# ioloizou/g1_locomotion

Hardware: AMD Instinct MI355X
Metric: QP solves/sec, SRBD N=10 12-state/12-input (higher is better)
Workload: dtype f64; 1 GPU; configs[1]: batch=4096/GPU random SRBD states, N=10, 2-contact alternating single support friction cone, fp64; tails deferred (SRBDQP_FLAG_DEFER_TAIL: the ~4 % of a batch that reach a rho-restart mark finish in the next launch on their stream; srbdqp_flush inside the timed region, every batch complete when the clock stops); steps rotate over 4 distinct device batches; horizon=10, batch_per_gpu=4096, kernel=wave_defer_f64_n10_s2, streams=2, longest_first_hint=False, deferred_tails=True, world_size=1, distinct_batches=4, max_iter=250, rho_restart_iter=0, rho_restart_count=0, set_up_dtype=f64

## Files before the change

g1_locomotion_amd/csrc/srbdqp_mfma.hpp:

```cpp
#pragma once
#include "srbdqp_common.hpp"
#include "srbdqp_admm.hpp"

namespace srbdqp {

constexpr bool kMfmaReady = true;

#ifdef SRBDQP_PROFILE_F
#define F_T(var) do { unsigned long long t_; asm volatile("s_memtime %0\n\ts_waitcnt lgkmcnt(0)" : "=s"(t_) :: "memory"); var = (long long)t_; } while (0)
#else
#define F_T(var) do { } while (0)
#endif

typedef double v4d __attribute__((ext_vector_type(4)));

__device__ __forceinline__ v4d mfma_f64(double a, double b, v4d c) {
    return __builtin_amdgcn_mfma_f64_16x16x4f64(a, b, c, 0, 0, 0);
}

__device__ __forceinline__ double readlane_f64(double v, int lane) {
    const int lo = __builtin_amdgcn_readlane(__double2loint(v), lane);
    const int hi = __builtin_amdgcn_readlane(__double2hiint(v), lane);
    return __hiloint2double(hi, lo);
}

__device__ __forceinline__ int tile_id(int a, int b) { return (b * (b + 1)) / 2 + a; }

template <bool SWZ>
__device__ __forceinline__ void store_tile(double* tile, const v4d& v, int lane) {
    const int col = lane & 15, g = lane >> 4;
#pragma unroll
    for (int r = 0; r < 4; ++r) {
        const int row = g + 4 * r;
        tile[row * 16 + (SWZ ? (col ^ row) : col)] = v[r];
    }
}

typedef float v4f __attribute__((ext_vector_type(4)));
__device__ __forceinline__ v4d mma16(double a, double b, v4d c) { return __builtin_amdgcn_mfma_f64_16x16x4f64(a, b, c, 0, 0, 0); }
__device__ __forceinline__ v4f mma16(float a, float b, v4f c) { return __builtin_amdgcn_mfma_f32_16x16x4f32(a, b, c, 0, 0, 0); }
template <typename TT> __device__ __forceinline__ int crow(int kq, int q) { return (sizeof(TT) == 8) ? kq + 4 * q : 4 * kq + q; }
template <typename TT, bool SWZ, typename V4>
__device__ __forceinline__ void store_tile_t(TT* tile, const V4& v, int lane) {
    const int col = lane & 15, g = lane >> 4;
#pragma unroll
    for (int q = 0; q < 4; ++q) {
        const int row = crow<TT>(g, q);
        tile[row * 16 + (SWZ ? (col ^ row) : col)] = v[q];
    }
}

__device__ __forceinline__ double fast_rsqrt(double d) {
    const double r = __builtin_amdgcn_rsq(d);
    const double h = 0.5 * d * r;
    return fma(r, fma(-h, r, 0.5), r);
}

__device__ __forceinline__ double fast_rsqrt2(double d) {
    double r = __builtin_amdgcn_rsq(d);
    double h = 0.5 * d * r;
    r = fma(r, fma(-h, r, 0.5), r);
    h = 0.5 * d * r;
    return fma(r, fma(-h, r, 0.5), r);
}

template <int KB>
__device__ __forceinline__ void diag16_block(v4d& s, v4d& rr, v4d& w, double& pmin, int lane) {
    const int col = lane & 15, k = lane >> 4, li = col & 3;
    const double sk = s[KB];
    const double d00 = readlane_f64(sk, 4 * KB), d01 = readlane_f64(sk, 4 * KB + 1), d02 = readlane_f64(sk, 4 * KB + 2), d03 = readlane_f64(sk, 4 * KB + 3);
    const double d11 = readlane_f64(sk, 16 + 4 * KB + 1), d12 = readlane_f64(sk, 16 + 4 * KB + 2), d13 = readlane_f64(sk, 16 + 4 * KB + 3);
    const double d22 = readlane_f64(sk, 32 + 4 * KB + 2), d23 = readlane_f64(sk, 32 + 4 * KB + 3);
    const double d33 = readlane_f64(sk, 48 + 4 * KB + 3);
    const double x00 = fast_rsqrt(d00);
    const double r01 = d01 * x00, r02 = d02 * x00, r03 = d03 * x00;
    const double p1 = fma(-r01, r01, d11);
    const double x11 = fast_rsqrt(p1);
    const double r12 = fma(-r01, r02, d12) * x11, r13 = fma(-r01, r03, d13) * x11;
    const double p2 = fma(-r12, r12, fma(-r02, r02, d22));
    const double x22 = fast_rsqrt(p2);
    const double r23 = fma(-r12, r13, fma(-r02, r03, d23)) * x22;
    const double p3 = fma(-r23, r23, fma(-r13, r13, fma(-r03, r03, d33)));
    const double x33 = fast_rsqrt(p3);
    pmin = (d00 > 0.0 && p1 > 0.0 && p2 > 0.0 && p3 > 0.0) ? pmin : -1.0;
    const double x01 = -x00 * r01 * x11;
    const double x12 = -x11 * r12 * x22;
    const double x23 = -x22 * r23 * x33;
    const double x02 = -fma(x00, r02, x01 * r12) * x22;
    const double x13 = -fma(x11, r13, x12 * r23) * x33;
    const double x03 = -fma(x00, r03, fma(x01, r13, x02 * r23)) * x33;
    const double c0 = x00;
    const double c1 = (k == 0) ? x01 : x11;
    const double c2 = (k == 0) ? x02 : (k == 1) ? x12 : x22;
    const double c3 = (k == 0) ? x03 : (k == 1) ? x13 : (k == 2) ? x23 : x33;
    double a = (li == 0) ? c0 : (li == 1) ? c1 : (li == 2) ? c2 : c3;
    a = (k <= li) ? a : 0.0;
    const v4d zero = (v4d){0.0, 0.0, 0.0, 0.0};
    double u = mfma_f64(a, sk, zero)[KB];
    u = (col >= 4 * KB) ? u : 0.0;
    const double wk = mfma_f64(a, rr[KB], zero)[KB];
    w[KB] = wk;
    if constexpr (KB < 3) {
        s = mfma_f64(-u, u, s);
        const double am = (col >= 4 * (KB + 1)) ? u : 0.0;
        rr = mfma_f64(-am, wk, rr);
        diag16_block<KB + 1>(s, rr, w, pmin, lane);
    }
}

__device__ __forceinline__ v4d diag16_invert_mfma(v4d s, int lane, bool& ok) {
    const int col = lane & 15, g = lane >> 4;
    v4d rr, w;
#pragma unroll
    for (int r = 0; r < 4; ++r) { rr[r] = (g + 4 * r == col) ? 1.0 : 0.0; w[r] = 0.0; }
    double pmin = 1.0e300;
    diag16_block<0>(s, rr, w, pmin, lane);
    ok = pmin > 0.0;
    return w;
}


template <int I>
__device__ __forceinline__ void fmac_newbcast(double& acc, double nu, double m) {
    asm("v_fmac_f64_dpp %0, %1, %2 row_newbcast:%3 row_mask:0xf bank_mask:0xf" : "+v"(acc) : "v"(nu), "v"(m), "n"(I));
}
template <int K>
__device__ __forceinline__ double mov_newbcast(double v) {
    double d;
    asm("s_nop 1\n\tv_mov_b64_dpp %0, %1 row_newbcast:%2 row_mask:0xf bank_mask:0xf" : "=v"(d) : "v"(v), "n"(K));
    return d;
}
template <int K, int I>
struct Diag16Rows {
    static __device__ __forceinline__ void run(double (&S)[16], double (&R)[16], double nu, double u, double wk) {
        if constexpr (I < 16) {
            fmac_newbcast<I>(S[I], nu, u);
            fmac_newbcast<I>(R[I], nu, wk);
            Diag16Rows<K, I + 1>::run(S, R, nu, u, wk);
        }
    }
};
template <int K, int KEND = 16>
__device__ __forceinline__ void diag16_pivot(double (&S)[16], double (&R)[16], bool& ok) {
    const double d = mov_newbcast<K>(S[K]);
    ok = ok && (d > 0.0);
    const double r = fast_rsqrt(d);
    const double u = S[K] * r;
    const double wk = R[K] * r;
    R[K] = wk;
    if constexpr (K < 15) {
        double nu;
        asm("v_mul_f64 %0, %1, %2\n\ts_nop 1" : "=v"(nu) : "v"(S[K]), "v"(-r));
        Diag16Rows<K, K + 1>::run(S, R, nu, u, wk);
    }
    if constexpr (K + 1 < KEND) diag16_pivot<K + 1, KEND>(S, R, ok);
}
__device__ __forceinline__ v4d diag16_invert_dpp(v4d s, int lane, bool& ok, double* tile) {
    const int col = lane & 15, g = lane >> 4;
    asm volatile("" ::: "memory");
#pragma unroll
    for (int r = 0; r < 4; ++r) tile[(g + 4 * r) * 16 + col] = s[r];
    asm volatile("" ::: "memory");
    double S[16], R[16];
#pragma unroll
    for (int i = 0; i < 16; ++i) { S[i] = tile[i * 16 + col]; R[i] = (i == col) ? 1.0 : 0.0; }
    asm volatile("" ::: "memory");
    ok = true;
    diag16_pivot<0>(S, R, ok);
    if (g == 0) {
#pragma unroll
        for (int i = 0; i < 16; ++i) tile[i * 16 + (col ^ i)] = R[i];
    }
    asm volatile("" ::: "memory");
    v4d w;
#pragma unroll
    for (int q = 0; q < 4; ++q) { const int row = g + 4 * q; w[q] = tile[row * 16 + (col ^ row)]; }
    asm volatile("" ::: "memory");
    return w;
}
template <typename TI, typename TO>
__device__ __forceinline__ void diag16_invert_dpp_tiles(const TI* in, TO* out, int lane, bool& ok) {
    const int col = lane & 15, g = lane >> 4;
    double S[16], R[16];
#pragma unroll
    for (int i = 0; i < 16; ++i) { S[i] = (double)in[i * 16 + col]; R[i] = (i == col) ? 1.0 : 0.0; }
    asm volatile("s_waitcnt lgkmcnt(0)" ::: "memory");
    ok = true;
    diag16_pivot<0>(S, R, ok);
    if (g == 0) {
#pragma unroll
        for (int i = 0; i < 16; ++i) out[i * 16 + (col ^ i)] = (TO)R[i];
    }
    asm volatile("" ::: "memory");
}

}
```

g1_locomotion_amd/csrc/srbdqp_setup1.hpp:

```cpp
#pragma once
#include "srbdqp_split.hpp"

namespace srbdqp {

#ifdef SRBDQP_WAVE_STAMPS
#define WSTAMP(a, b, idx) SRBDQP_STAMP(a, b, idx)
#define WSTAMP_RT(a, b, idx) do { if ((a).stamps && threadIdx.x == 0) (a).stamps[(size_t)(b) * 16 + (idx)] = (long long)__builtin_amdgcn_s_memrealtime(); } while (0)
#else
#define WSTAMP(a, b, idx) do { } while (0)
#define WSTAMP_RT(a, b, idx) do { } while (0)
#endif

template <int N, int MAXS>
struct Setup1Smem {
    using S = CompactSmem<N, MAXS>;
    static constexpr int n = Dims<N>::n;
    static constexpr int up2(int v) { return (v + 1) & ~1; }
    static constexpr int o_x0 = S::o_x0, o_tm = S::o_tm, o_J = S::o_J;
    static constexpr int o_cp = S::o_R;
    static constexpr int o_mt = o_cp + up2(9 * N);
    static constexpr int o_ab = o_mt + 18 * N;
    static constexpr int o_gv = o_mt + up2(9 * S::NPAIR);
    static constexpr int o_t1 = o_gv + up2(9 * N);
    static constexpr int o_t2 = o_t1 + up2(9 * N);
    static constexpr int o_x0c = o_t1;
    static constexpr int o_tf = o_x0c + up2(S::nmax) + 16;
    static constexpr int endT = (o_t2 + up2(9 * N) > o_tf + 6 * N) ? o_t2 + up2(9 * N) : o_tf + 6 * N;
    static constexpr int o_xref = up2(endT);
    static constexpr int o_foot = o_xref + up2(N * 13);
    static constexpr int o_pcom = o_foot + N * 12;
    static constexpr int o_eh = o_foot;
    static constexpr int o_gx = o_foot;
    static constexpr int o_scr = o_xref;
    static constexpr int endIn = o_pcom + up2(N * 3);
    static constexpr int endIn2 = (endIn > o_scr + 258) ? endIn : o_scr + 258;
    static constexpr int kStgRow = 18;
    static constexpr int kStgTile = 16 * kStgRow;
    static constexpr int endStg = (endIn2 > o_cp + S::NT * kStgTile) ? endIn2 : o_cp + S::NT * kStgTile;
    static constexpr int endAb = o_ab + 16 * S::NT * kAbStride;
    static constexpr int o_end = endStg > endAb ? endStg : endAb;
    static constexpr size_t bytes = (size_t)o_end * sizeof(double);
    static constexpr bool supported = SplitWs<N, MAXS>::supported && S::NT <= 4;
    static_assert(n + 6 * N <= o_end - o_eh || true, "");
};

template <int N, int MAXS, bool FUSED, bool DUMP, bool PHI, int RP>
__device__ __forceinline__ bool setup1_pass(const KArgs& a, const QpIo& io, const int b, double* sm, double& rho_b, int& rs_pass, int& rs_done) {
    using S = CompactSmem<N, MAXS>;
    using W = SplitWs<N, MAXS>;
    using L1 = Setup1Smem<N, MAXS>;
    constexpr int n = Dims<N>::n, m = Dims<N>::m, NT = S::NT;
    int lane = threadIdx.x;
    if constexpr (RP == 2) asm volatile("" : "+v"(lane));
    [[maybe_unused]] double* const park = sm + L1::o_end;
    int mcol = lane & 15, kq = lane >> 4;
    double* ws = FUSED ? nullptr : a.ws + (size_t)b * W::doubles;
    int* icnt = reinterpret_cast<int*>(sm + S::o_int);
    int* imisc = icnt + 2 * N;
    uint8_t* act = reinterpret_cast<uint8_t*>(imisc + 8);
    uint8_t* sct = reinterpret_cast<uint8_t*>(sm + S::o_ct);
    const double* SQ = sm + S::o_sq;
    const double* CP = sm + L1::o_cp;

    WSTAMP(a, b, 0);
    WSTAMP_RT(a, b, 12);
    constexpr int JT = (12 * N + 63) / 64;
    double yc, ys;
    [[maybe_unused]] double v_xr[JT];
    if constexpr (RP == 2) {
        const int k = lane < N ? lane : 0;
        yc = sm[S::o_tm + k * 9 + 0];
        ys = sm[S::o_tm + k * 9 + 1];
    } else {
        const double* gx0 = io.x0 + (size_t)b * 13;
        const double* gxr = io.xref + (size_t)b * N * 13;
        const double* gft = io.foot + (size_t)b * N * 12;
        const uint8_t* gct = io.contact + (size_t)b * N * 4;
        const double* gpc = io.pcom ? io.pcom + (size_t)b * N * 3 : nullptr;
        const double v_x0 = gx0[lane < 13 ? lane : 0];
        const uint8_t v_ct = gct[lane < 4 * N ? lane : 0];
        const double v_yaw = gxr[(lane < N ? lane : 0) * 13 + 2];
        double v_f[JT][3], v_p[JT][3];
#pragma unroll
        for (int t = 0; t < JT; ++t) {
            const int tt = (lane + 64 * t < 12 * N) ? lane + 64 * t : 0;
            const int k = tt / 12, ci = (tt % 12) / 3;
            const double* pc = gpc ? gpc + k * 3 : gxr + k * 13 + 3;
#pragma unroll
            for (int c = 0; c < 3; ++c) { v_f[t][c] = gft[k * 12 + 3 * ci + c]; v_p[t][c] = pc[c]; }
            v_xr[t] = gxr[k * 13 + (tt - 12 * k)];
        }
        sincos(v_yaw, &ys, &yc);
        if (lane < 13) sm[S::o_x0 + lane] = v_x0;
        if (lane >= 32 && lane < 44) sm[S::o_sq + lane - 32] = a.sqrtq[lane - 32];
        if (lane < N * 4) sct[lane] = v_ct ? 1 : 0;
        if (lane < N) {
            double* T = sm + S::o_tm + lane * 9;
            T[0] = yc;  T[1] = ys;  T[2] = 0.0;
            T[3] = -ys; T[4] = yc;  T[5] = 0.0;
            T[6] = 0.0; T[7] = 0.0; T[8] = 1.0;
        }
        {
            const bool flag = (lane < 4 * N) && v_ct != 0;
            const unsigned long long bal = __ballot(flag);
            if (flag) act[__popcll(bal & ((1ull << lane) - 1ull))] = (uint8_t)lane;
            if (lane < N) icnt[lane] = __popcll(bal & ((4 * (lane + 1) >= 64) ? ~0ull : ((1ull << (4 * (lane + 1))) - 1ull)));
            const bool over = lane < N && __popcll((bal >> (4 * (lane < N ? lane : 0))) & 0xFull) > MAXS;
            const unsigned long long viol = __ballot(over);
            if (lane == 0) {
                imisc[0] = __popcll(bal);
                imisc[1] = viol != 0ull;
                sm[S::o_misc] = 0.0;
                sm[S::o_misc + 1] = 0.0;
            }
        }
#pragma unroll
        for (int t = 0; t < JT; ++t) {
            const int tt = lane + 64 * t;
            const int k = (tt < 12 * N ? tt : 0) / 12, cc = tt - 12 * k, ax = cc % 3;
            const double cs = __shfl(yc, k), sn = __shfl(ys, k);
            const double i0 = a.iinv[0], i1 = a.iinv[1], i2 = a.iinv[2];
            const double w00 = cs * cs * i0 + sn * sn * i1, w01 = cs * sn * (i0 - i1), w11 = sn * sn * i0 + cs * cs * i1;
            const double rx = v_f[t][0] - v_p[t][0];
            const double ry = v_f[t][1] - v_p[t][1];
            const double rz = v_f[t][2] - v_p[t][2];
            const double s0 = (ax == 0) ? 0.0 : ((ax == 1) ? -rz : ry);
            const double s1 = (ax == 0) ? rz : ((ax == 1) ? 0.0 : -rx);
            const double s2 = (ax == 0) ? -ry : ((ax == 1) ? rx : 0.0);
            if (tt < 12 * N) {
                double* J = sm + S::o_J + k * 36;
                J[0 * 12 + cc] = w00 * s0 + w01 * s1;
                J[1 * 12 + cc] = w01 * s0 + w11 * s1;
                J[2 * 12 + cc] = i2 * s2;
            }
        }
    }
    double ccu[N], csu[N], ccm = 0.0, csm = 0.0;
    {
        double ac = 0.0, as = 0.0;
#pragma unroll
        for (int k = 0; k < N; ++k) {
            const double c = lane_bcast(yc, k), s = lane_bcast(ys, k);
            ac += c;
            as += s;
            ccu[k] = ac;
            csu[k] = as;
            ccm += (k <= lane) ? c : 0.0;
            csm += (k <= lane) ? s : 0.0;
        }
    }
    if (lane < N) {
        double* C = sm + L1::o_cp + lane * 9;
        C[0] = ccm;  C[1] = csm; C[2] = 0.0;
        C[3] = -csm; C[4] = ccm; C[5] = 0.0;
        C[6] = 0.0;  C[7] = 0.0; C[8] = (double)(lane + 1);
    }
    __syncthreads();
    const int na = imisc[0];
    const int n_eff = 3 * na;
    double* xs0 = sm + L1::o_mt;
    static_assert(L1::o_end - L1::o_mt >= n + 12 * N, "early-exit scratch");
    if (RP != 2 && (imisc[1] != 0 || na == 0)) {
        if constexpr (DUMP) { if (lane == 0) a.ub_out[(size_t)b * m] = (imisc[1] != 0) ? -1.0 : 0.0; return false; }
        for (int c = lane; c < n; c += 64) xs0[c] = 0.0;
        if (io.y_out) for (int i = lane; i < m; i += 64) io.y_out[(size_t)b * m + i] = 0.0;
        if (lane == 0) {
            if (io.status) io.status[b] = (imisc[1] != 0) ? kStatusContactBound : 1;
            if (io.iters) io.iters[b] = a.iters_base;
            if constexpr (!FUSED) ws[S::o_misc + 1] = 1.0;
        }
        __syncthreads();
        rollout_and_store_to<N, S, 64>(a, io.u_out, io.x_out, b, sm, xs0, xs0 + n);
        return false;
    }

    WSTAMP(a, b, 1);
    const double dt = a.dt, dt2 = a.dt * a.dt, dtm = a.dt * a.inv_mass, dt2m = dt2 * a.inv_mass;
    double* DE = sm + L1::o_mt;
    double* GV = sm + L1::o_gv;
    if constexpr (RP != 2) {
#pragma unroll
        for (int t = 0; t < JT; ++t) {
            const int k = lane + 64 * t;
            const int kc = k < n ? k : 0, i = kc / 12, kk = kc - 12 * i;
            const double v = SQ[kk] * (free_response_sel<N, L1>(a, sm, i, kk) - v_xr[t]);
            if (k < n) sm[L1::o_eh + k] = v;
        }
    }
    if (lane < N) {
        const int mm = lane;
        const double w0 = SQ[0] * SQ[0], w1 = SQ[1] * SQ[1], w2 = SQ[2] * SQ[2];
        double t1a = 0.0, t1b = 0.0, t2aa = 0.0, t2ab = 0.0, t2bb = 0.0, t2zz = 0.0;
#pragma unroll
        for (int i = 0; i < N; ++i) {
            const bool on = i >= mm;
            const double da = ccu[i] - ccm, db = csu[i] - csm, dz = (double)(i - mm);
            t1a += on ? da : 0.0;
            t1b += on ? db : 0.0;
            t2aa += on ? (w0 * da) * da + (w1 * db) * db : 0.0;
            t2ab += on ? (w0 * da) * db - (w1 * db) * da : 0.0;
            t2bb += on ? (w0 * db) * db + (w1 * da) * da : 0.0;
            t2zz += on ? (w2 * dz) * dz : 0.0;
        }
        const double t1z = (double)(((N - mm) * (N - mm - 1)) / 2);
        const double Cm[9] = {ccm, csm, 0.0, -csm, ccm, 0.0, 0.0, 0.0, (double)(mm + 1)};
        const double t1[9] = {t1a, t1b, 0.0, -t1b, t1a, 0.0, 0.0, 0.0, t1z};
        const double t2[9] = {t2aa, t2ab, 0.0, t2ab, t2bb, 0.0, 0.0, 0.0, t2zz};
        de_step<N>(Cm, t1, t2, SQ, dt2, mm, DE + 18 * mm);
    }
    auto gt_tables = [&](const double* vec) {
        for (int e = lane; e < 3 * N; e += 64) {
            const int j = e / 3, comp = e - 3 * j;
            const double* Cj = CP + j * 9;
            double acc = 0.0;
#pragma unroll
            for (int i = 0; i < N; ++i) {
                const double* Ci = CP + i * 9;
                const double* v = vec + 12 * i;
                const double term = dt2 * ((Ci[comp] - Cj[comp]) * (SQ[0] * v[0]) + (Ci[3 + comp] - Cj[3 + comp]) * (SQ[1] * v[1]) +
                                           (Ci[6 + comp] - Cj[6 + comp]) * (SQ[2] * v[2])) + dt * (SQ[6 + comp] * v[6 + comp]);
                acc += (i >= j) ? term : 0.0;
            }
            GV[9 * j + comp] = acc;
        }
        constexpr int HL = (3 * N) % 64;
        for (int e = lane - HL; e < 6 * N; e += 64) {
            if (e < 0) continue;
            const int j = e / 6, comp = 3 + (e - 6 * j);
            double acc = 0.0;
            const int off = (comp < 6) ? comp : 3 + comp;
#pragma unroll
            for (int i = 0; i < N; ++i) {
                const double v = vec[12 * i + off];
                const double term = (comp < 6) ? (double)(i - j) * v : v;
                acc += (i >= j) ? term : 0.0;
            }
            GV[9 * j + comp] = acc;
        }
    };
    auto gt_eval = [&](int c) -> double {
        const int e = c / 3, ax = c - 3 * e, gc = act[e], j = gc >> 2;
        const double* J = sm + S::o_J + j * 36 + 3 * (gc & 3) + ax;
        const double* g = GV + 9 * j;
        return a.s * (J[0] * g[0] + J[12] * g[1] + J[24] * g[2] + SQ[3 + ax] * dt2m * g[3 + ax] + SQ[9 + ax] * dtm * g[6 + ax]);
    };
    __syncthreads();
    if constexpr (RP != 2) gt_tables(sm + L1::o_eh);
    __syncthreads();
    WSTAMP(a, b, 2);
    if constexpr (RP != 2) for (int c = lane; c < n_eff; c += 64) sm[S::o_q + c] = gt_eval(c);
    if (RP >= 2 || a.warm_u) {
        double* TF = sm + L1::o_tf;
        for (int c = lane; c < n_eff; c += 64)
            sm[L1::o_x0c + c] = (RP >= 2 ? park[c] : a.warm_u[(size_t)b * n + 3 * act[c / 3] + (c % 3)]) / a.s;
        __syncthreads();
        for (int tt = lane; tt < 6 * N; tt += 64) {
            const int j = tt / 6, comp = tt - 6 * j;
            double acc = 0.0;
            for (int e = (j ? icnt[j - 1] : 0); e < icnt[j]; ++e) {
                const double* x = sm + L1::o_x0c + 3 * e;
                if (comp < 3) {
                    const double* J = sm + S::o_J + j * 36 + comp * 12 + 3 * (act[e] & 3);
                    acc += J[0] * x[0] + J[1] * x[1] + J[2] * x[2];
                } else {
                    acc += x[comp - 3];
                }
            }
            TF[tt] = acc;
        }
        __syncthreads();
        for (int k = lane; k < n; k += 64) {
            const int i = k / 12, kk = k - 12 * i;
            const double acc = gx_row<N>(CP, TF, i, kk, dt, dt2, dtm, dt2m);
            sm[L1::o_gx + k] = SQ[kk] * a.s * acc;
        }
        __syncthreads();
        gt_tables(sm + L1::o_gx);
        __syncthreads();
        for (int c = lane; c < n_eff; c += 64) sm[S::o_px0 + c] = gt_eval(c) + a.rs2 * sm[L1::o_x0c + c];
    } else {
        for (int c = lane; c < n_eff; c += 64) sm[S::o_px0 + c] = 0.0;
    }

    if constexpr (PHI) {
        double* phi = ws + W::o_phi;
        const double x0_keep = (lane < 13) ? sm[S::o_x0 + lane] : 0.0;
        for (int kc = 0; kc < 13; ++kc) {
            __syncthreads();
            if (lane < 13) sm[S::o_x0 + lane] = (lane == kc) ? 1.0 : 0.0;
            __syncthreads();
            for (int k = lane; k < n; k += 64) {
                const int i = k / 12, kk = k - 12 * i;
                sm[L1::o_eh + k] = SQ[kk] * free_response<N, L1>(a, sm, i, kk);
            }
            __syncthreads();
            gt_tables(sm + L1::o_eh);
            __syncthreads();
            for (int c = lane; c < n_eff; c += 64) phi[c * 13 + kc] = gt_eval(c);
        }
        __syncthreads();
        if (lane < 13) sm[S::o_x0 + lane] = x0_keep;
        __syncthreads();
    }
    WSTAMP(a, b, 3);
    v4d Kt[NT][NT];
    __syncthreads();
    {
        double* AB = sm + L1::o_ab;
        kasm_rows<N>(sm + S::o_J, CP, DE, SQ, act, n_eff, a.s, dt2m, dtm, AB, lane, 64, 16 * NT);
        __syncthreads();
        typedef double d2 __attribute__((ext_vector_type(2)));
        const double dgxy = uni(a.rs2 + a.sigma + 2.0 * rho_b), dgz = uni(a.rs2 + a.sigma + (4.0 * a.mu * a.mu + a.rho_fz) * rho_b);
        const int d3 = (mcol - kq + 3) % 3;
        const double ind[3] = {d3 == 0 ? 1.0 : 0.0, d3 == 1 ? 1.0 : 0.0, d3 == 2 ? 1.0 : 0.0};
        double eqd[4];
#pragma unroll
        for (int q = 0; q < 4; ++q) eqd[q] = (kq + 4 * q == mcol) ? 1.0 : 0.0;
        double Bv[NT][8], dcol[NT];
#pragma unroll
        for (int tb = 0; tb < NT; ++tb) {
            const int c = 16 * tb + mcol;
            const d2* row = reinterpret_cast<const d2*>(AB + kAbStride * c + 8);
#pragma unroll
            for (int i = 0; i < 4; ++i) { const d2 v = row[i]; Bv[tb][2 * i] = v[0]; Bv[tb][2 * i + 1] = v[1]; }
            dcol[tb] = (c < n_eff) ? (((tb + mcol) % 3 < 2) ? dgxy : dgz) : 1.0;
        }
#pragma unroll
        for (int ta = 0; ta < NT; ++ta) {
#pragma unroll
            for (int q = 0; q < 4; ++q) {
                const int r = 16 * ta + kq + 4 * q;
                const d2* row = reinterpret_cast<const d2*>(AB + kAbStride * r);
                double Av[8];
#pragma unroll
                for (int i = 0; i < 4; ++i) { const d2 v = row[i]; Av[2 * i] = v[0]; Av[2 * i + 1] = v[1]; }
#pragma unroll
                for (int tb = ta; tb < NT; ++tb) {
                    double v = Av[0] * Bv[tb][0];
#pragma unroll
                    for (int i = 1; i < 6; ++i) v = fma(Av[i], Bv[tb][i], v);
                    const double ft = fma(Av[7], Bv[tb][7], Av[6] * Bv[tb][6]);
                    v = fma(ind[((ta + q - tb) % 3 + 3) % 3], ft, v);
                    if (ta == tb) v = fma(eqd[q], dcol[tb], v);
                    Kt[ta][tb][q] = v;
                }
            }
        }
    }
    __syncthreads();
    WSTAMP(a, b, 4);
    WSTAMP(a, b, 5);
    if constexpr (DUMP) {
        dump_presolved<N>(a, b, n_eff, na, sm + S::o_q, act, [&](auto&& put) {
#pragma unroll
            for (int ta = 0; ta < NT; ++ta)
#pragma unroll
                for (int tb = ta; tb < NT; ++tb)
#pragma unroll
                    for (int q = 0; q < 4; ++q)
                        if (16 * ta + kq + 4 * q <= 16 * tb + mcol) put(16 * ta + kq + 4 * q, 16 * tb + mcol, Kt[ta][tb][q]);
        });
        return false;
    }

    double* scr = sm + L1::o_scr;
    auto a_operand = [&](const v4d& x, double (&op)[4]) {
        asm volatile("" ::: "memory");
#pragma unroll
        for (int q = 0; q < 4; ++q) {
            const int row = kq + 4 * q;
            scr[row * 16 + (mcol ^ row)] = x[q];
        }
        asm volatile("" ::: "memory");
#pragma unroll
        for (int r = 0; r < 4; ++r) op[r] = scr[mcol * 16 + ((4 * r + kq) ^ mcol)];
        asm volatile("" ::: "memory");
    };
    const v4d zero4 = (v4d){0.0, 0.0, 0.0, 0.0};

    bool all_ok = true;
#pragma unroll
    for (int j = 0; j < NT; ++j) {
        bool ok;
        v4d w = diag16_invert_mfma(Kt[j][j], lane, ok);
        all_ok = all_ok && ok;
#pragma unroll
        for (int q = 0; q < 4; ++q) w[q] = (mcol <= kq + 4 * q) ? w[q] : 0.0;
        Kt[j][j] = w;
        if (j + 1 < NT) {
            double wa[4];
            a_operand(w, wa);
#pragma unroll
            for (int bb = j + 1; bb < NT; ++bb) {
                v4d o = zero4;
#pragma unroll
                for (int r = 0; r < 4; ++r) o = mfma_f64(wa[r], Kt[j][bb][r], o);
                Kt[j][bb] = o;
            }
#pragma unroll
            for (int aa = j + 1; aa < NT; ++aa)
#pragma unroll
                for (int bb = aa; bb < NT; ++bb)
#pragma unroll
                    for (int r = 0; r < 4; ++r) Kt[aa][bb] = mfma_f64(-Kt[j][aa][r], Kt[j][bb][r], Kt[aa][bb]);
        }
    }
    if (!all_ok && lane == 0) sm[S::o_misc] = 1.0;
    WSTAMP(a, b, 6);

#pragma unroll
    for (int i = 1; i < NT; ++i) {
        double wa[4];
        a_operand(Kt[i][i], wa);
#pragma unroll
        for (int j = 0; j < i; ++j) {
            v4d sacc = zero4;
#pragma unroll
            for (int k = j; k < i; ++k) {
                const v4d& wkj = (k == j) ? Kt[j][j] : Kt[j][k];
#pragma unroll
                for (int r = 0; r < 4; ++r) sacc = mfma_f64(Kt[k][i][r], wkj[r], sacc);
            }
            v4d o = zero4;
#pragma unroll
            for (int r = 0; r < 4; ++r) o = mfma_f64(-wa[r], sacc[r], o);
            Kt[j][i] = o;
        }
    }

    WSTAMP(a, b, 7);
    double kin[W::KS];
    if constexpr (!FUSED) {
        for (int i = lane; i < S::o_R; i += 64) ws[i] = sm[i];
        double* kinv = ws + W::o_kinv;
#pragma unroll
        for (int aa = 0; aa < NT; ++aa) {
#pragma unroll
            for (int bb = aa; bb < NT; ++bb) {
                v4d o = zero4;
#pragma unroll
                for (int k = bb; k < NT; ++k) {
                    const v4d& wka = (k == aa) ? Kt[aa][aa] : Kt[aa][k];
                    const v4d& wkb = (k == bb) ? Kt[bb][bb] : Kt[bb][k];
#pragma unroll
                    for (int r = 0; r < 4; ++r) o = mfma_f64(wka[r], wkb[r], o);
                }
                const int col = 16 * bb + mcol;
#pragma unroll
                for (int q = 0; q < 4; ++q) {
                    const int row = 16 * aa + kq + 4 * q;
                    if (row < n_eff && col < W::KS) kinv[row * W::KS + col] = (col < n_eff) ? o[q] : 0.0;
                    if (aa != bb && col < n_eff && row < W::KS) kinv[col * W::KS + row] = (row < n_eff) ? o[q] : 0.0;
                }
            }
        }
    } else {
        double* stg = sm + L1::o_cp;
        static_assert(L1::o_end - L1::o_cp >= NT * L1::kStgTile, "staging of one block column of K^-1");
        const int grp = lane >> 4;
        v4d Ku[NT][NT];
#pragma unroll
        for (int cb = NT - 1; cb >= 0; --cb) {
            asm volatile("" ::: "memory");
#pragma unroll
            for (int g = 0; g <= cb; ++g) {
                v4d o = zero4;
#pragma unroll
                for (int k = cb; k < NT; ++k) {
                    const v4d& wkg = (k == g) ? Kt[g][g] : Kt[g][k];
                    const v4d& wkc = (k == cb) ? Kt[cb][cb] : Kt[cb][k];
#pragma unroll
                    for (int r = 0; r < 4; ++r) o = mfma_f64(wkg[r], wkc[r], o);
                }
#pragma unroll
                for (int q = 0; q < 4; ++q) stg[g * L1::kStgTile + (kq + 4 * q) * L1::kStgRow + mcol] = o[q];
                if (g < cb) Ku[g][cb] = o;
            }
#pragma unroll
            for (int g = cb + 1; g < NT; ++g)
#pragma unroll
                for (int q = 0; q < 4; ++q) stg[g * L1::kStgTile + mcol * L1::kStgRow + kq + 4 * q] = Ku[cb][g][q];
            asm volatile("" ::: "memory");
            const double2* rowp = reinterpret_cast<const double2*>(stg + grp * L1::kStgTile + mcol * L1::kStgRow);
#pragma unroll
            for (int h = 0; h < 8; ++h) {
                if (16 * cb + 2 * h + 1 < W::KS + 1) {
                    const double2 v = rowp[h];
                    if (16 * cb + 2 * h < W::KS) kin[16 * cb + 2 * h] = v.x;
                    if (16 * cb + 2 * h + 1 < W::KS) kin[16 * cb + 2 * h + 1] = v.y;
                }
            }
            asm volatile("" ::: "memory");
        }
    }
    if constexpr (FUSED) {
        if (__builtin_amdgcn_readfirstlane(n_eff) < W::KS) {
#pragma unroll
            for (int c = 0; c < W::KS; ++c) kin[c] = (lane < n_eff && c < n_eff) ? kin[c] : 0.0;
        }
        __syncthreads();
        WSTAMP(a, b, 8);
        WSTAMP(a, b, 9);
        static_assert(L1::o_end >= SplitSmem<N, MAXS>::o_end, "the ADMM body's vectors live in this kernel's LDS");
        if constexpr (RP == 0) {
            admm_wave_body<N, MAXS>(a, b, rho_b, sm, kin);
        } else {
            WaveRestart rs;
            const int left = a.max_iter - rs_done;
            rs.pass = rs_pass;
            rs.more = rs_pass < a.restart_max && a.restart_every < left;
            rs.kcap = rs.more ? a.restart_every : left;
            rs.park = park;
            int status = -1, iters = 0;
            admm_wave_iterations<N, MAXS, true>(a, io, RP == 1 ? a.warm_u : nullptr, RP == 1 ? a.warm_y : nullptr, b, rho_b, sm, kin, sm + SplitSmem<N, MAXS>::o_xs,
                                                status, iters, &rs);
            rs_done += iters;
            if (status == 2 && rs.more) {
                rho_b = restart_rho_of(rho_b, rs.v);
                ++rs_pass;
                __syncthreads();
                return true;
            }
            admm_wave_finish<N, MAXS>(a, io, b, sm, status, rs_done);
        }
        WSTAMP(a, b, 10);
        WSTAMP(a, b, 11);
        WSTAMP_RT(a, b, 13);
    }
    return false;
}

template <int N, int MAXS, bool FUSED, bool DUMP = false, bool PHI = false, bool RST = false>
__global__ __launch_bounds__(64, 2) void srbdqp_setup1_kernel(KArgs a) {
    static_assert(!(PHI && FUSED), "dq/dx0 is a hand-over of the split pipeline");
    static_assert(!RST || (FUSED && !DUMP), "the restart in place belongs to the fused solve");
    static_assert(Setup1Smem<N, MAXS>::supported, "one wave holds all tiles: at most 4 x 4 tiles");
    static_assert(4 * N <= 64, "one ballot compacts the contact flags");
    extern __shared__ __attribute__((aligned(16))) double sm[];
    if ((int)blockIdx.x >= a.B) return;
    if (a.count_ptr && (int)blockIdx.x >= *a.count_ptr) return;
    const int b = SRBDQP_QP_INDEX(a);
    if (SRBDQP_RESTART_SKIP(a, b)) return;
    double rho_b = SRBDQP_RHO_OF(a, b);
    int rs_pass = 0, rs_done = 0;
    const QpIo io = io_of(a);
    if constexpr (!RST) {
        setup1_pass<N, MAXS, FUSED, DUMP, PHI, 0>(a, io, b, sm, rho_b, rs_pass, rs_done);
    } else {
        bool again = setup1_pass<N, MAXS, FUSED, DUMP, PHI, 1>(a, io, b, sm, rho_b, rs_pass, rs_done);
        if (!again) return;
        again = setup1_pass<N, MAXS, FUSED, DUMP, PHI, 2>(a, io, b, sm, rho_b, rs_pass, rs_done);
        if (!again) return;
        again = setup1_pass<N, MAXS, FUSED, DUMP, PHI, 2>(a, io, b, sm, rho_b, rs_pass, rs_done);
        if (!again) return;
        KArgs al = a;
        al.restart_max = 0;
        setup1_pass<N, MAXS, FUSED, DUMP, PHI, 2>(al, io, b, sm, rho_b, rs_pass, rs_done);
    }
}

__device__ __forceinline__ unsigned long long unis_u64(unsigned long long v) {
    int lo, hi;
    asm volatile("s_nop 1\n\tv_readfirstlane_b32 %0, %2\n\tv_readfirstlane_b32 %1, %3" : "=s"(lo), "=s"(hi) : "v"((int)(unsigned)v), "v"((int)(unsigned)(v >> 32)));
    return ((unsigned long long)(unsigned)hi << 32) | (unsigned long long)(unsigned)lo;
}
template <typename T> __device__ __forceinline__ T* unis_ptr(T* p) { return reinterpret_cast<T*>(unis_u64(reinterpret_cast<unsigned long long>(p))); }

__device__ __forceinline__ double* tail_claim(const KArgs& a) {
    int slot = 0;
    if (threadIdx.x == 0) slot = atomicAdd(a.tail_cnt + a.tail_iout, 1);
    slot = __builtin_amdgcn_readfirstlane(slot);
    if (slot >= a.tail_cap) return nullptr;
    return reinterpret_cast<double*>(a.tail_lists) + ((size_t)a.tail_iout * (size_t)a.tail_cap + (size_t)slot) * kTailRecDoubles;
}

__device__ __forceinline__ bool tail_export(const KArgs& a, const QpIo& io, int b, double rho_b, int rs_pass, int rs_done, const double* park) {
    const int lane = threadIdx.x;
    double* rec = tail_claim(a);
    if (!rec) return false;
    if (lane == 0) {
        TailRecHead* hd = reinterpret_cast<TailRecHead*>(rec);
        hd->b = b; hd->pass = rs_pass; hd->done = rs_done; hd->pad = 0; hd->rho = rho_b; hd->io = io;
        if (io.status) io.status[b] = kStatusPending;
    }
    rec[16 + lane] = park[lane]; rec[80 + lane] = park[64 + lane]; rec[144 + lane] = park[128 + lane];
    return true;
}

template <int N, int MAXS, bool FLUSH = false>
__global__ __launch_bounds__(64, 2) void srbdqp_wave_defer_kernel(KArgs a) {
    static_assert(Setup1Smem<N, MAXS>::supported && 4 * N <= 64, "the one-wave kernel's limits");
    extern __shared__ __attribute__((aligned(16))) double sm[];
    using L1 = Setup1Smem<N, MAXS>;
    const int lane = threadIdx.x;
    const int T = a.tail_wgs;
    double* const park = sm + L1::o_end;
    auto in_place = [&](const QpIo& io, const int b, double rho_b, int rs_pass, int rs_done) __attribute__((always_inline)) {
        bool again = setup1_pass<N, MAXS, true, false, false, 2>(a, io, b, sm, rho_b, rs_pass, rs_done);
        if (!again) return;
        again = setup1_pass<N, MAXS, true, false, false, 2>(a, io, b, sm, rho_b, rs_pass, rs_done);
        if (!again) return;
        KArgs al = a;
        al.restart_max = 0;
        setup1_pass<N, MAXS, true, false, false, 2>(al, io, b, sm, rho_b, rs_pass, rs_done);
    };
    if ((int)blockIdx.x < T) {
        const int i = blockIdx.x;
        int cnt = a.tail_cnt[a.tail_iin];
        cnt = cnt < a.tail_cap ? cnt : a.tail_cap;
        if (i == 0 && lane == 0) a.tail_cnt[a.tail_izero] = 0;
        const double* lin = reinterpret_cast<const double*>(a.tail_lists) + (size_t)a.tail_iin * (size_t)a.tail_cap * kTailRecDoubles;
        if (i >= cnt) return;
        const double* rec = lin + (size_t)i * kTailRecDoubles;
        const TailRecHead* hd = reinterpret_cast<const TailRecHead*>(rec);
        QpIo io;
        io.x0 = unis_ptr(hd->io.x0); io.xref = unis_ptr(hd->io.xref); io.foot = unis_ptr(hd->io.foot); io.pcom = unis_ptr(hd->io.pcom);
        io.contact = unis_ptr(hd->io.contact); io.u_out = unis_ptr(hd->io.u_out); io.x_out = unis_ptr(hd->io.x_out); io.y_out = unis_ptr(hd->io.y_out);
        io.status = unis_ptr(hd->io.status); io.iters = unis_ptr(hd->io.iters);
        const int b = __builtin_amdgcn_readfirstlane(hd->b);
        int rs_pass = __builtin_amdgcn_readfirstlane(hd->pass), rs_done = __builtin_amdgcn_readfirstlane(hd->done);
        double rho_b = unis(hd->rho);
        park[lane] = rec[16 + lane]; park[64 + lane] = rec[80 + lane]; park[128 + lane] = rec[144 + lane];
        __syncthreads();
        if (!setup1_pass<N, MAXS, true, false, false, 3>(a, io, b, sm, rho_b, rs_pass, rs_done)) return;
        if constexpr (!FLUSH) { if (tail_export(a, io, b, rho_b, rs_pass, rs_done, park)) return; }
        in_place(io, b, rho_b, rs_pass, rs_done);
    } else if constexpr (!FLUSH) {
        const int wg = (int)blockIdx.x - T;
        if (wg >= a.B) return;
        const int b = a.perm ? a.perm[wg] : wg;
        double rho_b = a.rho_qp ? a.rho_qp[b] : a.rho;
        int rs_pass = 0, rs_done = 0;
        const QpIo io = io_of(a);
        if (!setup1_pass<N, MAXS, true, false, false, 1>(a, io, b, sm, rho_b, rs_pass, rs_done)) return;
        if (tail_export(a, io, b, rho_b, rs_pass, rs_done, park)) return;
        in_place(io, b, rho_b, rs_pass, rs_done);
    }
}

}
```

Baseline: 38.87 million QP/s.

## Replace MFMA diagonal-block inverse Cholesky with packed DPP row-broadcast elimination

The 16x16 diagonal-block inverse-Cholesky in setup now uses a packed DPP variant instead of the blocked MFMA path. Each lane pair holds the matrix column and its identity column, joined with permlane16 swaps, and the elimination runs through v_fmac_f64_dpp row_newbcast chains. Positive-definiteness is checked through the high word of the exponent. The inverse is written to the scratch tile already swizzled, so the next operand read reuses it instead of doing another store and masking pass. The goal is to cut MFMA latency chains and readlane traffic in the serial factorization, at the cost of intricate hand-written asm and a slightly different pivot-failure test.

```diff
diff --git a/g1_locomotion_amd/csrc/srbdqp_mfma.hpp b/g1_locomotion_amd/csrc/srbdqp_mfma.hpp
--- a/g1_locomotion_amd/csrc/srbdqp_mfma.hpp
+++ b/g1_locomotion_amd/csrc/srbdqp_mfma.hpp
@@ -178,6 +178,120 @@
     asm volatile("" ::: "memory");
     return w;
 }
+__device__ __forceinline__ double pk_even_rows(double x) {
+    int alo, ahi, blo, bhi;
+    asm("v_mov_b32 %0, %4\n\tv_mov_b32 %2, %4\n\tv_mov_b32 %1, %5\n\tv_mov_b32 %3, %5\n\ts_nop 1\n\t"
+        "v_permlane16_swap_b32 %0, %2\n\tv_permlane16_swap_b32 %1, %3"
+        : "=&v"(alo), "=&v"(ahi), "=&v"(blo), "=&v"(bhi) : "v"(__double2loint(x)), "v"(__double2hiint(x)));
+    return __hiloint2double(ahi, alo);
+}
+#define SRBDQP_PK(P, I) "v_fmac_f64_dpp %" #P ", %8, %9 row_newbcast:" #I " row_mask:0xf bank_mask:0xf\n\t"
+#define SRBDQP_PK_LO7 SRBDQP_PK(7, 7)
+#define SRBDQP_PK_LO6 SRBDQP_PK(6, 6) SRBDQP_PK_LO7
+#define SRBDQP_PK_LO5 SRBDQP_PK(5, 5) SRBDQP_PK_LO6
+#define SRBDQP_PK_LO4 SRBDQP_PK(4, 4) SRBDQP_PK_LO5
+#define SRBDQP_PK_LO3 SRBDQP_PK(3, 3) SRBDQP_PK_LO4
+#define SRBDQP_PK_LO2 SRBDQP_PK(2, 2) SRBDQP_PK_LO3
+#define SRBDQP_PK_HI15 SRBDQP_PK(7, 15)
+#define SRBDQP_PK_HI14 SRBDQP_PK(6, 14) SRBDQP_PK_HI15
+#define SRBDQP_PK_HI13 SRBDQP_PK(5, 13) SRBDQP_PK_HI14
+#define SRBDQP_PK_HI12 SRBDQP_PK(4, 12) SRBDQP_PK_HI13
+#define SRBDQP_PK_HI11 SRBDQP_PK(3, 11) SRBDQP_PK_HI12
+#define SRBDQP_PK_HI10 SRBDQP_PK(2, 10) SRBDQP_PK_HI11
+#define SRBDQP_PK_HI9 SRBDQP_PK(1, 9) SRBDQP_PK_HI10
+#define SRBDQP_PK_HI8 SRBDQP_PK(0, 8) SRBDQP_PK_HI9
+#define SRBDQP_PK_ASM(TAIL, B) asm("s_nop 1\n\t" TAIL : "+v"(X[B]), "+v"(X[B + 1]), "+v"(X[B + 2]), "+v"(X[B + 3]), "+v"(X[B + 4]), "+v"(X[B + 5]), "+v"(X[B + 6]), "+v"(X[B + 7]) : "v"(nu), "v"(y))
+template <int FROM>
+__device__ __forceinline__ void pk_rows(double (&X)[16], double nu, double y) {
+    if constexpr (FROM == 2) SRBDQP_PK_ASM(SRBDQP_PK_LO2, 0);
+    else if constexpr (FROM == 3) SRBDQP_PK_ASM(SRBDQP_PK_LO3, 0);
+    else if constexpr (FROM == 4) SRBDQP_PK_ASM(SRBDQP_PK_LO4, 0);
+    else if constexpr (FROM == 5) SRBDQP_PK_ASM(SRBDQP_PK_LO5, 0);
+    else if constexpr (FROM == 6) SRBDQP_PK_ASM(SRBDQP_PK_LO6, 0);
+    else if constexpr (FROM == 7) SRBDQP_PK_ASM(SRBDQP_PK_LO7, 0);
+    if constexpr (FROM <= 8) SRBDQP_PK_ASM(SRBDQP_PK_HI8, 8);
+    else if constexpr (FROM == 9) SRBDQP_PK_ASM(SRBDQP_PK_HI9, 8);
+    else if constexpr (FROM == 10) SRBDQP_PK_ASM(SRBDQP_PK_HI10, 8);
+    else if constexpr (FROM == 11) SRBDQP_PK_ASM(SRBDQP_PK_HI11, 8);
+    else if constexpr (FROM == 12) SRBDQP_PK_ASM(SRBDQP_PK_HI12, 8);
+    else if constexpr (FROM == 13) SRBDQP_PK_ASM(SRBDQP_PK_HI13, 8);
+    else if constexpr (FROM == 14) SRBDQP_PK_ASM(SRBDQP_PK_HI14, 8);
+    else if constexpr (FROM == 15) SRBDQP_PK_ASM(SRBDQP_PK_HI15, 8);
+}
+#undef SRBDQP_PK_ASM
+#undef SRBDQP_PK_HI8
+#undef SRBDQP_PK_HI9
+#undef SRBDQP_PK_HI10
+#undef SRBDQP_PK_HI11
+#undef SRBDQP_PK_HI12
+#undef SRBDQP_PK_HI13
+#undef SRBDQP_PK_HI14
+#undef SRBDQP_PK_HI15
+#undef SRBDQP_PK_LO2
+#undef SRBDQP_PK_LO3
+#undef SRBDQP_PK_LO4
+#undef SRBDQP_PK_LO5
+#undef SRBDQP_PK_LO6
+#undef SRBDQP_PK_LO7
+#undef SRBDQP_PK
+template <int I>
+struct PkLoad {
+    static __device__ __forceinline__ void run(double (&X)[16], const double* colp, int one_hi) {
+        if constexpr (I < 16) {
+            const double t = colp[I * 16];
+            const int lo = __builtin_amdgcn_update_dpp(__double2loint(t), 0, 0xE4, 0xA, 0xF, false);
+            const int hi = __builtin_amdgcn_update_dpp(__double2hiint(t), one_hi, I == 0 ? 0xE4 : 0x110 + I, 0xA, 0xF, true);
+            X[I] = __hiloint2double(hi, lo);
+            PkLoad<I + 1>::run(X, colp, one_hi);
+        }
+    }
+};
+template <int K>
+__device__ __forceinline__ void diag16_pivot_packed(double (&X)[16], unsigned& worst) {
+    const double sk = pk_even_rows(X[K]);
+    const double d = mov_newbcast<K>(sk);
+    const unsigned dh = (unsigned)__double2hiint(d) - 1u;
+    worst = dh > worst ? dh : worst;
+    const double r = fast_rsqrt(d);
+    const double y = X[K] * r;
+    if constexpr (K < 15) {
+        double nu;
+        asm("v_mul_f64 %1, %3, -%4\n\ts_nop 1\n\tv_fmac_f64_dpp %0, %1, %2 row_newbcast:%5 row_mask:0xf bank_mask:0xf"
+            : "+v"(X[K + 1]), "=&v"(nu) : "v"(y), "v"(sk), "v"(r), "n"(K + 1));
+        if constexpr (K < 14) pk_rows<K + 2>(X, nu, y);
+        X[K] = y;
+        diag16_pivot_packed<K + 1>(X, worst);
+    } else {
+        X[K] = y;
+    }
+}
+__device__ __forceinline__ v4d diag16_invert_dpp_packed(v4d s, int lane, bool& ok, double* tile) {
+    const int col = lane & 15, g = lane >> 4;
+    asm volatile("" ::: "memory");
+#pragma unroll
+    for (int r = 0; r < 4; ++r) tile[(g + 4 * r) * 16 + col] = s[r];
+    asm volatile("" ::: "memory");
+    const int one_hi = (col == 0) ? 0x3ff00000 : 0;
+    double X[16];
+    PkLoad<0>::run(X, tile + col, one_hi);
+    asm volatile("" ::: "memory");
+    unsigned worst = 0u;
+    diag16_pivot_packed<0>(X, worst);
+    ok = worst < 0x7fefffffu;
+    int colw = col;
+    asm("" : "+v"(colw) : "v"(X[15]));
+    if (g == 1) {
+#pragma unroll
+        for (int i = 0; i < 16; ++i) tile[i * 16 + (colw ^ i)] = X[i];
+    }
+    asm volatile("" ::: "memory");
+    v4d w;
+#pragma unroll
+    for (int q = 0; q < 4; ++q) { const int row = g + 4 * q; w[q] = tile[row * 16 + (col ^ row)]; }
+    asm volatile("" ::: "memory");
+    return w;
+}
+
 template <typename TI, typename TO>
 __device__ __forceinline__ void diag16_invert_dpp_tiles(const TI* in, TO* out, int lane, bool& ok) {
     const int col = lane & 15, g = lane >> 4;
diff --git a/g1_locomotion_amd/csrc/srbdqp_setup1.hpp b/g1_locomotion_amd/csrc/srbdqp_setup1.hpp
--- a/g1_locomotion_amd/csrc/srbdqp_setup1.hpp
+++ b/g1_locomotion_amd/csrc/srbdqp_setup1.hpp
@@ -364,6 +364,11 @@
     }
 
     double* scr = sm + L1::o_scr;
+    auto a_operand_read = [&](double (&op)[4]) {
+#pragma unroll
+        for (int r = 0; r < 4; ++r) op[r] = scr[mcol * 16 + ((4 * r + kq) ^ mcol)];
+        asm volatile("" ::: "memory");
+    };
     auto a_operand = [&](const v4d& x, double (&op)[4]) {
         asm volatile("" ::: "memory");
 #pragma unroll
@@ -372,9 +377,7 @@
             scr[row * 16 + (mcol ^ row)] = x[q];
         }
         asm volatile("" ::: "memory");
-#pragma unroll
-        for (int r = 0; r < 4; ++r) op[r] = scr[mcol * 16 + ((4 * r + kq) ^ mcol)];
-        asm volatile("" ::: "memory");
+        a_operand_read(op);
     };
     const v4d zero4 = (v4d){0.0, 0.0, 0.0, 0.0};
 
@@ -382,14 +385,12 @@
 #pragma unroll
     for (int j = 0; j < NT; ++j) {
         bool ok;
-        v4d w = diag16_invert_mfma(Kt[j][j], lane, ok);
+        const v4d w = diag16_invert_dpp_packed(Kt[j][j], lane, ok, scr);
         all_ok = all_ok && ok;
-#pragma unroll
-        for (int q = 0; q < 4; ++q) w[q] = (mcol <= kq + 4 * q) ? w[q] : 0.0;
         Kt[j][j] = w;
         if (j + 1 < NT) {
             double wa[4];
-            a_operand(w, wa);
+            a_operand_read(wa);
 #pragma unroll
             for (int bb = j + 1; bb < NT; ++bb) {
                 v4d o = zero4;
```

Result: faster. 40.17 million QP/s, median of 6 (+3.4%).
